# adamchang2000/DenseFusion

Measured on AMD Instinct MI355X. Metric: poses/sec (node) YCB-Video 1000 pts + 2 refine iters, higher is better.
Workload: dtype f32

## Files before the change

densefusion_amd/csrc/split_gemm.hip:

```cpp
#include "igemm.h"
#include <atomic>
#include <cstdint>
#ifdef DF_DEV
#include <map>
#include <mutex>
#include <tuple>
#endif

namespace df {
namespace {

typedef __bf16 bf16x8 __attribute__((ext_vector_type(8)));
typedef __bf16 bf16x2 __attribute__((ext_vector_type(2)));
typedef float f32x16 __attribute__((ext_vector_type(16)));
typedef float f32x2 __attribute__((ext_vector_type(2)));

constexpr int SBM = 128, SBN = 128, SBK = 32;
constexpr int PLANE_BYTES = 128 * 64;

__device__ __forceinline__ void cut3(float a0, float a1, unsigned &hi, unsigned &mid, unsigned &lo) {
  const bf16x2 h = __builtin_convertvector(f32x2{a0, a1}, bf16x2);
  hi = __builtin_bit_cast(unsigned, h);
  const float r0 = a0 - __builtin_bit_cast(float, hi << 16), r1 = a1 - __builtin_bit_cast(float, hi & 0xFFFF0000u);
  const bf16x2 m = __builtin_convertvector(f32x2{r0, r1}, bf16x2);
  mid = __builtin_bit_cast(unsigned, m);
  const float s0 = r0 - __builtin_bit_cast(float, mid << 16), s1 = r1 - __builtin_bit_cast(float, mid & 0xFFFF0000u);
  const bf16x2 l = __builtin_convertvector(f32x2{s0, s1}, bf16x2);
  lo = __builtin_bit_cast(unsigned, l);
}

__global__ void cut_planes_kernel(const float *__restrict__ w, __bf16 *__restrict__ planes, long elems, long stride) {
  const long i = (long)blockIdx.x * blockDim.x + threadIdx.x;
  if (i >= elems) return;
  unsigned h, m, l;
  cut3(w[i], 0.f, h, m, l);
  unsigned short *pl = reinterpret_cast<unsigned short *>(planes);
  pl[i] = (unsigned short)h; pl[stride + i] = (unsigned short)m; pl[2 * stride + i] = (unsigned short)l;
}

struct SplitArgs {
  const float *in; const __bf16 *wpl; const float *bias; const float *res; const float *prelu; float *out; float *colsum;
  long M, wplane;
  int N, K, in_ld, in_coff, out_ld, out_coff, res_ld, res_coff, act, rows_per_group, rows_valid, bias_group_ld;
  long z_in_coff, z_wgt, z_bias, z_out_coff;
  int tiles_m, tiles_n;
  long cs_rows;
};

__device__ __forceinline__ int piece(int row, int slot) { return row * 64 + ((slot ^ ((row >> 2) & 3)) << 4); }

__device__ __forceinline__ void split_epilogue(const SplitArgs &a, const f32x16 (&acc)[2][2], int z, long row0, int wrow, int nb, int fr, int fh, long cs_row) {
  const float slope = a.act == ACT_PRELU ? a.prelu[0] : 0.f;
  float *out = a.out + z * a.z_out_coff + a.out_coff;
  const float *bias = a.bias ? a.bias + z * a.z_bias : nullptr;
  const float *gbias = bias && a.bias_group_ld > 0 ? bias + (row0 / a.rows_per_group) * a.bias_group_ld : nullptr;
  const int grp = a.rows_per_group > 0 ? (int)(row0 / a.rows_per_group) : 0;
  const long left = a.M - row0;
  const int valid = a.rows_per_group > 0 ? a.rows_valid - (int)(row0 - (long)grp * a.rows_per_group) : (1 << 30);
  const int limit = (int)(left < valid ? left : valid);
#pragma unroll
  for (int j = 0; j < 2; ++j) {
    const int n = nb + j * 32 + fr;
    const float b1 = gbias ? gbias[n] : bias ? bias[n] : 0.f;
    float csum = 0.f;
#pragma unroll
    for (int i = 0; i < 2; ++i) {
      const int tb = wrow + i * 32 + 4 * fh;
      const long mb = row0 + tb;
      float r[16];
      if (a.res) {
#pragma unroll
        for (int e = 0; e < 16; ++e) {
          long m = mb + (e & 3) + 8 * (e >> 2);
          m = m < a.M ? m : a.M - 1;
          r[e] = a.res[m * a.res_ld + a.res_coff + n];
        }
      }
#pragma unroll
      for (int e = 0; e < 16; ++e) {
        const int tr = tb + (e & 3) + 8 * (e >> 2);
        const long m = row0 + tr;
        float v = acc[i][j][e] + b1;
        if (a.res) v += r[e];
        if (a.act == ACT_RELU) v = v > 0.f ? v : 0.f;
        else if (a.act == ACT_PRELU) v = v > 0.f ? v : v * slope;
        if (a.out && m < a.M) out[m * a.out_ld + n] = v;
        csum += tr < limit ? v : 0.f;
      }
    }
    if (a.colsum && cs_row < a.cs_rows) {
      csum += __shfl_xor(csum, 32);
      if (fh == 0) a.colsum[((size_t)z * a.cs_rows + (size_t)cs_row) * a.N + n] = csum;
    }
  }
}

__device__ __forceinline__ void split_epilogue_rows(const SplitArgs &a, const f32x16 (&acc)[2][2], int z, long row0, int wrow, int nb, int lane, long cs_row, float *blk) {
  const int fr = lane & 31, fh = lane >> 5;
  const float slope = a.act == ACT_PRELU ? a.prelu[0] : 0.f;
  const float *bias = a.bias ? a.bias + z * a.z_bias : nullptr;
  const float *gbias = bias && a.bias_group_ld > 0 ? bias + (row0 / a.rows_per_group) * a.bias_group_ld : nullptr;
  const int grp = a.rows_per_group > 0 ? (int)(row0 / a.rows_per_group) : 0;
  const long left = a.M - row0;
  const int valid = a.rows_per_group > 0 ? a.rows_valid - (int)(row0 - (long)grp * a.rows_per_group) : (1 << 30);
  const int limit = (int)(left < valid ? left : valid);
#pragma unroll
  for (int j = 0; j < 2; ++j) {
    const int n = nb + j * 32 + fr;
    const float b1 = gbias ? gbias[n] : bias ? bias[n] : 0.f;
    float csum = 0.f;
#pragma unroll
    for (int i = 0; i < 2; ++i)
#pragma unroll
      for (int e = 0; e < 16; ++e) {
        const int br = i * 32 + 4 * fh + (e & 3) + 8 * (e >> 2);
        float v = acc[i][j][e] + b1;
        if (!a.res) {
          if (a.act == ACT_RELU) v = v > 0.f ? v : 0.f;
          else if (a.act == ACT_PRELU) v = v > 0.f ? v : v * slope;
        }
        blk[br * 64 + j * 32 + fr] = v;
        csum += wrow + br < limit ? v : 0.f;
      }
    if (a.colsum && cs_row < a.cs_rows) {
      csum += __shfl_xor(csum, 32);
      if (fh == 0) a.colsum[((size_t)z * a.cs_rows + (size_t)cs_row) * a.N + n] = csum;
    }
  }
  if (!a.out) return;
  __builtin_amdgcn_fence(__ATOMIC_RELEASE, "wavefront");
  __builtin_amdgcn_wave_barrier();
  __builtin_amdgcn_fence(__ATOMIC_ACQUIRE, "wavefront");
  float *out = a.out + z * a.z_out_coff + a.out_coff;
  const int c4 = (lane & 15) * 4;
#pragma unroll 4
  for (int it = 0; it < 16; ++it) {
    const int br = it * 4 + (lane >> 4);
    const long m = row0 + wrow + br;
    float4 v = *reinterpret_cast<const float4 *>(blk + br * 64 + c4);
    if (m < a.M) {
      if (a.res) {
        const float4 r = *reinterpret_cast<const float4 *>(a.res + m * a.res_ld + a.res_coff + nb + c4);
        v.x += r.x; v.y += r.y; v.z += r.z; v.w += r.w;
        if (a.act == ACT_RELU) {
          v.x = v.x > 0.f ? v.x : 0.f; v.y = v.y > 0.f ? v.y : 0.f; v.z = v.z > 0.f ? v.z : 0.f; v.w = v.w > 0.f ? v.w : 0.f;
        } else if (a.act == ACT_PRELU) {
          v.x = v.x > 0.f ? v.x : v.x * slope; v.y = v.y > 0.f ? v.y : v.y * slope; v.z = v.z > 0.f ? v.z : v.z * slope; v.w = v.w > 0.f ? v.w : v.w * slope;
        }
      }
      *reinterpret_cast<float4 *>(out + m * a.out_ld + nb + c4) = v;
    }
  }
  __builtin_amdgcn_fence(__ATOMIC_RELEASE, "wavefront");
  __builtin_amdgcn_wave_barrier();
}

__global__ __launch_bounds__(256, 2) void gemm_split_bf16_kernel(const SplitArgs a) {
  __shared__ __attribute__((aligned(16))) unsigned char lds[6 * PLANE_BYTES];
  const int tid = threadIdx.x, lane = tid & 63, wave = tid >> 6;
  const int xcd = blockIdx.x & 7, seq = blockIdx.x >> 3;
  const int tm = (seq / a.tiles_n) * 8 + xcd, tn = seq % a.tiles_n;
  if (tm >= a.tiles_m) return;
  const int z = blockIdx.z;
  const long row0 = (long)tm * SBM;
  const int n0 = tn * SBN;
  const float *in = a.in + z * a.z_in_coff + a.in_coff;
  const __bf16 *wpl = a.wpl + z * a.z_wgt;

  const int srow0 = tid >> 2, srow1 = srow0 + 64, sslot = tid & 3;
  const int soff0 = piece(srow0, sslot), soff1 = piece(srow1, sslot);
  long r0 = row0 + srow0, r1 = row0 + srow1;
  r0 = r0 < a.M ? r0 : a.M - 1;
  r1 = r1 < a.M ? r1 : a.M - 1;
  const float *ag0 = in + r0 * a.in_ld + sslot * 8, *ag1 = in + r1 * a.in_ld + sslot * 8;
  const __bf16 *bg0 = wpl + (long)(n0 + srow0) * a.K + sslot * 8, *bg1 = wpl + (long)(n0 + srow1) * a.K + sslot * 8;
  float4 xa00, xa01, xa10, xa11, ya00, ya01, ya10, ya11;
  uint4 rb00, rb01, rb02, rb10, rb11, rb12;
#define SPLIT_FETCH_A(S, k0)                                                     \
  do {                                                                           \
    S##a00 = *reinterpret_cast<const float4 *>(ag0 + (k0));                      \
    S##a01 = *reinterpret_cast<const float4 *>(ag0 + (k0) + 4);                  \
    S##a10 = *reinterpret_cast<const float4 *>(ag1 + (k0));                      \
    S##a11 = *reinterpret_cast<const float4 *>(ag1 + (k0) + 4);                  \
  } while (0)
#define SPLIT_FETCH_B(k0)                                                        \
  do {                                                                           \
    rb00 = *reinterpret_cast<const uint4 *>(bg0 + (k0));                         \
    rb01 = *reinterpret_cast<const uint4 *>(bg0 + a.wplane + (k0));              \
    rb02 = *reinterpret_cast<const uint4 *>(bg0 + 2 * a.wplane + (k0));          \
    rb10 = *reinterpret_cast<const uint4 *>(bg1 + (k0));                         \
    rb11 = *reinterpret_cast<const uint4 *>(bg1 + a.wplane + (k0));              \
    rb12 = *reinterpret_cast<const uint4 *>(bg1 + 2 * a.wplane + (k0));          \
  } while (0)
#define SPLIT_STAGE1(x0, x1, off, b0, b1, b2)                                    \
  do {                                                                           \
    uint4 h, m, l;                                                               \
    cut3(x0.x, x0.y, h.x, m.x, l.x);                                             \
    cut3(x0.z, x0.w, h.y, m.y, l.y);                                             \
    cut3(x1.x, x1.y, h.z, m.z, l.z);                                             \
    cut3(x1.z, x1.w, h.w, m.w, l.w);                                             \
    *reinterpret_cast<uint4 *>(lds + (off)) = h;                                 \
    *reinterpret_cast<uint4 *>(lds + PLANE_BYTES + (off)) = m;                   \
    *reinterpret_cast<uint4 *>(lds + 2 * PLANE_BYTES + (off)) = l;               \
    *reinterpret_cast<uint4 *>(lds + 3 * PLANE_BYTES + (off)) = b0;              \
    *reinterpret_cast<uint4 *>(lds + 4 * PLANE_BYTES + (off)) = b1;              \
    *reinterpret_cast<uint4 *>(lds + 5 * PLANE_BYTES + (off)) = b2;              \
  } while (0)
#define SPLIT_STAGE(S)                                                           \
  do {                                                                           \
    SPLIT_STAGE1(S##a00, S##a01, soff0, rb00, rb01, rb02);                       \
    SPLIT_STAGE1(S##a10, S##a11, soff1, rb10, rb11, rb12);                       \
  } while (0)

  const int wr = wave >> 1, wc = wave & 1, fr = lane & 31, fh = lane >> 5;
  f32x16 acc[2][2];
#pragma unroll
  for (int i = 0; i < 2; ++i)
#pragma unroll
    for (int j = 0; j < 2; ++j)
#pragma unroll
      for (int e = 0; e < 16; ++e) acc[i][j][e] = 0.f;
  int offa[2][2], offb[2][2];
#pragma unroll
  for (int ks = 0; ks < 2; ++ks)
#pragma unroll
    for (int t = 0; t < 2; ++t) {
      offa[ks][t] = piece(wr * 64 + t * 32 + fr, ks * 2 + fh);
      offb[ks][t] = 3 * PLANE_BYTES + piece(wc * 64 + t * 32 + fr, ks * 2 + fh);
    }

#define SPLIT_COMPUTE()                                                                                   \
  _Pragma("unroll") for (int ks = 0; ks < 2; ++ks) {                                                      \
    bf16x8 fa[2][3], fb[2][3];                                                                            \
    _Pragma("unroll") for (int t = 0; t < 2; ++t)                                                         \
    _Pragma("unroll") for (int p = 0; p < 3; ++p) {                                                       \
      fa[t][p] = *reinterpret_cast<const bf16x8 *>(lds + p * PLANE_BYTES + offa[ks][t]);                  \
      fb[t][p] = *reinterpret_cast<const bf16x8 *>(lds + p * PLANE_BYTES + offb[ks][t]);                  \
    }                                                                                                     \
    _Pragma("unroll") for (int i = 0; i < 2; ++i)                                                         \
    _Pragma("unroll") for (int j = 0; j < 2; ++j) {                                                       \
      f32x16 c = acc[i][j];                                                        \
      c = __builtin_amdgcn_mfma_f32_32x32x16_bf16(fa[i][2], fb[j][0], c, 0, 0, 0);                        \
      c = __builtin_amdgcn_mfma_f32_32x32x16_bf16(fa[i][0], fb[j][2], c, 0, 0, 0);                        \
      c = __builtin_amdgcn_mfma_f32_32x32x16_bf16(fa[i][1], fb[j][1], c, 0, 0, 0);                        \
      c = __builtin_amdgcn_mfma_f32_32x32x16_bf16(fa[i][1], fb[j][0], c, 0, 0, 0);                        \
      c = __builtin_amdgcn_mfma_f32_32x32x16_bf16(fa[i][0], fb[j][1], c, 0, 0, 0);                        \
      c = __builtin_amdgcn_mfma_f32_32x32x16_bf16(fa[i][0], fb[j][0], c, 0, 0, 0);                        \
      acc[i][j] = c;                                                                                      \
    }                                                                                                     \
  }

  const int nk = a.K / SBK;
  SPLIT_FETCH_A(x, 0);
  SPLIT_FETCH_B(0);
  if (nk > 1) SPLIT_FETCH_A(y, SBK);
  SPLIT_STAGE(x);
  __syncthreads();
  for (int kt = 0; kt < nk; kt += 2) {
    if (kt + 1 < nk) SPLIT_FETCH_B((kt + 1) * SBK);
    if (kt + 2 < nk) SPLIT_FETCH_A(x, (kt + 2) * SBK);
    SPLIT_COMPUTE();
    if (kt + 1 >= nk) break;
    __syncthreads();
    SPLIT_STAGE(y);
    __syncthreads();
    if (kt + 2 < nk) SPLIT_FETCH_B((kt + 2) * SBK);
    if (kt + 3 < nk) SPLIT_FETCH_A(y, (kt + 3) * SBK);
    SPLIT_COMPUTE();
    if (kt + 2 >= nk) break;
    __syncthreads();
    SPLIT_STAGE(x);
    __syncthreads();
  }

  split_epilogue(a, acc, z, row0, wr * 64, n0 + wc * 64, fr, fh, (long)tm * 2 + wr);
}

constexpr int V2_APL = 256 * 64, V2_BPL = 128 * 64, V2_STAGE = 3 * V2_APL + 3 * V2_BPL;

__global__ __launch_bounds__(512, 1) void gemm_split_bf16_v2_kernel(const SplitArgs a) {
  extern __shared__ __attribute__((aligned(16))) unsigned char lds2[];
  const int tid = threadIdx.x, lane = tid & 63, wave = tid >> 6;
  const int xcd = blockIdx.x & 7, seq = blockIdx.x >> 3;
  const int tm = (seq / a.tiles_n) * 8 + xcd, tn = seq % a.tiles_n;
  if (tm >= a.tiles_m) return;
  const int z = blockIdx.z;
  const long row0 = (long)tm * 256;
  const int n0 = tn * SBN;
  const float *in = a.in + z * a.z_in_coff + a.in_coff;
  const __bf16 *wpl = a.wpl + z * a.z_wgt;

  const int srow0 = tid >> 2, srow1 = srow0 + 128, sslot = tid & 3;
  const int soff0 = piece(srow0, sslot), soff1 = piece(srow1, sslot);
  long r0 = row0 + srow0, r1 = row0 + srow1;
  r0 = r0 < a.M ? r0 : a.M - 1;
  r1 = r1 < a.M ? r1 : a.M - 1;
  const float *ag0 = in + r0 * a.in_ld + sslot * 8, *ag1 = in + r1 * a.in_ld + sslot * 8;
  const __bf16 *bg0 = wpl + (long)(n0 + srow0) * a.K + sslot * 8;
  float4 xa00, xa01, xa10, xa11, ya00, ya01, ya10, ya11;
  uint4 xb0, xb1, xb2, yb0, yb1, yb2;
#define V2_FETCH(S, k0)                                                          \
  do {                                                                           \
    S##a00 = *reinterpret_cast<const float4 *>(ag0 + (k0));                      \
    S##a01 = *reinterpret_cast<const float4 *>(ag0 + (k0) + 4);                  \
    S##a10 = *reinterpret_cast<const float4 *>(ag1 + (k0));                      \
    S##a11 = *reinterpret_cast<const float4 *>(ag1 + (k0) + 4);                  \
    S##b0 = *reinterpret_cast<const uint4 *>(bg0 + (k0));                        \
    S##b1 = *reinterpret_cast<const uint4 *>(bg0 + a.wplane + (k0));             \
    S##b2 = *reinterpret_cast<const uint4 *>(bg0 + 2 * a.wplane + (k0));         \
  } while (0)
#define V2_CUT(x0, x1, base, off)                                                \
  do {                                                                           \
    uint4 h, m, l;                                                               \
    cut3(x0.x, x0.y, h.x, m.x, l.x);                                             \
    cut3(x0.z, x0.w, h.y, m.y, l.y);                                             \
    cut3(x1.x, x1.y, h.z, m.z, l.z);                                             \
    cut3(x1.z, x1.w, h.w, m.w, l.w);                                             \
    *reinterpret_cast<uint4 *>((base) + (off)) = h;                              \
    *reinterpret_cast<uint4 *>((base) + V2_APL + (off)) = m;                     \
    *reinterpret_cast<uint4 *>((base) + 2 * V2_APL + (off)) = l;                 \
  } while (0)
#define V2_STAGE_TO(S, base)                                                     \
  do {                                                                           \
    V2_CUT(S##a00, S##a01, base, soff0);                                         \
    V2_CUT(S##a10, S##a11, base, soff1);                                         \
    *reinterpret_cast<uint4 *>((base) + 3 * V2_APL + soff0) = S##b0;             \
    *reinterpret_cast<uint4 *>((base) + 3 * V2_APL + V2_BPL + soff0) = S##b1;    \
    *reinterpret_cast<uint4 *>((base) + 3 * V2_APL + 2 * V2_BPL + soff0) = S##b2; \
  } while (0)

  const int wr = wave >> 1, wc = wave & 1, fr = lane & 31, fh = lane >> 5;
  f32x16 acc[2][2];
#pragma unroll
  for (int i = 0; i < 2; ++i)
#pragma unroll
    for (int j = 0; j < 2; ++j)
#pragma unroll
      for (int e = 0; e < 16; ++e) acc[i][j][e] = 0.f;
  int offa[2][2], offb[2][2];
#pragma unroll
  for (int ks = 0; ks < 2; ++ks)
#pragma unroll
    for (int t = 0; t < 2; ++t) {
      offa[ks][t] = piece(wr * 64 + t * 32 + fr, ks * 2 + fh);
      offb[ks][t] = 3 * V2_APL + piece(wc * 64 + t * 32 + fr, ks * 2 + fh);
    }
#define V2_COMPUTE(base)                                                                                  \
  _Pragma("unroll") for (int ks = 0; ks < 2; ++ks) {                                                      \
    bf16x8 fa[2][3], fb[2][3];                                                                            \
    _Pragma("unroll") for (int t = 0; t < 2; ++t)                                                         \
    _Pragma("unroll") for (int p = 0; p < 3; ++p) {                                                       \
      fa[t][p] = *reinterpret_cast<const bf16x8 *>((base) + p * V2_APL + offa[ks][t]);                    \
      fb[t][p] = *reinterpret_cast<const bf16x8 *>((base) + p * V2_BPL + offb[ks][t]);                    \
    }                                                                                                     \
    _Pragma("unroll") for (int q = 0; q < 6; ++q) {                                                       \
      constexpr int PA[6] = {2, 0, 1, 1, 0, 0}, PB[6] = {0, 2, 1, 0, 1, 0};                               \
      _Pragma("unroll") for (int i = 0; i < 2; ++i)                                                       \
      _Pragma("unroll") for (int j = 0; j < 2; ++j)                                                       \
        acc[i][j] = __builtin_amdgcn_mfma_f32_32x32x16_bf16(fa[i][PA[q]], fb[j][PB[q]], acc[i][j], 0, 0, 0); \
    }                                                                                                     \
  }
#define V2_BODY(FS, SS, kf, cur, nxt)                                            \
  do {                                                                           \
    V2_FETCH(FS, (kf));                                                          \
    V2_STAGE_TO(SS, nxt);                                                        \
    V2_COMPUTE(cur);                                                             \
    __builtin_amdgcn_sched_group_barrier(0x020, 7, 0);                           \
    __builtin_amdgcn_sched_group_barrier(0x100, 12, 0);                          \
    _Pragma("unroll") for (int g = 0; g < 48; ++g) {                             \
      __builtin_amdgcn_sched_group_barrier(0x008, 1, 0);                         \
      __builtin_amdgcn_sched_group_barrier(0x002, 2, 0);                         \
      if (g >= 8 && g < 32 && (g & 1) == 0) __builtin_amdgcn_sched_group_barrier(0x100, 1, 0); \
      if (g % 5 == 4) __builtin_amdgcn_sched_group_barrier(0x200, 1, 0);         \
    }                                                                            \
    __syncthreads();                                                             \
  } while (0)

  unsigned char *const st0 = lds2, *const st1 = lds2 + V2_STAGE;
  const int nk = a.K / SBK;
  const int klast = a.K - SBK;
  V2_FETCH(x, 0);
  V2_FETCH(y, SBK < klast ? SBK : klast);
  V2_STAGE_TO(x, st0);
  __syncthreads();
  int kt = 0;
  for (; kt + 1 < nk; kt += 2) {
    const int k2 = (kt + 2) * SBK, k3 = (kt + 3) * SBK;
    V2_BODY(x, y, k2 < klast ? k2 : klast, st0, st1);
    V2_BODY(y, x, k3 < klast ? k3 : klast, st1, st0);
  }
  if (nk & 1) { V2_COMPUTE(st0); }
  split_epilogue(a, acc, z, row0, wr * 64, n0 + wc * 64, fr, fh, (long)tm * 4 + wr);
}

constexpr int V3_PL = 256 * 32, V3_STAGE = 6 * V3_PL;
constexpr int V3_LDS = 8 * 64 * 64 * 4;

__device__ __forceinline__ int piece16(int row, int half) { return row * 32 + ((half ^ ((row >> 3) & 1)) << 4); }

__global__ __launch_bounds__(512, 1) void gemm_split_bf16_v3_kernel(const SplitArgs a) {
  extern __shared__ __attribute__((aligned(16))) unsigned char lds3[];
  const int tid = threadIdx.x, lane = tid & 63, wave = tid >> 6;
  const int xcd = blockIdx.x & 7, seq = blockIdx.x >> 3;
  const int tm = (seq / a.tiles_n) * 8 + xcd, tn = seq % a.tiles_n;
  if (tm >= a.tiles_m) return;
  const int z = blockIdx.z;
  const long row0 = (long)tm * 256;
  const int n0 = tn * 256;
  const float *in = a.in + z * a.z_in_coff + a.in_coff;
  const __bf16 *wpl = a.wpl + z * a.z_wgt;

  const int srow = tid >> 1, shalf = tid & 1;
  const int soff = piece16(srow, shalf);
  long r = row0 + srow;
  r = r < a.M ? r : a.M - 1;
  const float *ag = in + r * a.in_ld + shalf * 8;
  const __bf16 *bg = wpl + (long)(n0 + srow) * a.K + shalf * 8;
  float4 xa0, xa1, ya0, ya1;
  uint4 b0, b1, b2;
#define V3_FETCH_A(S, k0)                                                        \
  do {                                                                           \
    S##a0 = *reinterpret_cast<const float4 *>(ag + (k0));                        \
    S##a1 = *reinterpret_cast<const float4 *>(ag + (k0) + 4);                    \
  } while (0)
#define V3_FETCH_B(k0)                                                           \
  do {                                                                           \
    b0 = *reinterpret_cast<const uint4 *>(bg + (k0));                            \
    b1 = *reinterpret_cast<const uint4 *>(bg + a.wplane + (k0));                 \
    b2 = *reinterpret_cast<const uint4 *>(bg + 2 * a.wplane + (k0));             \
  } while (0)
#define V3_PIN(v) asm volatile("" : "+v"(v.x), "+v"(v.y), "+v"(v.z), "+v"(v.w))
#define V3_CUT0(S) do { V3_PIN(S##a0); cut3(S##a0.x, S##a0.y, ch.x, cm.x, cl.x); cut3(S##a0.z, S##a0.w, ch.y, cm.y, cl.y); } while (0)
#define V3_CUT1(S) do { V3_PIN(S##a1); cut3(S##a1.x, S##a1.y, ch.z, cm.z, cl.z); cut3(S##a1.z, S##a1.w, ch.w, cm.w, cl.w); } while (0)
#define V3_WRITE_A(base)                                                         \
  do {                                                                           \
    *reinterpret_cast<uint4 *>((base) + soff) = ch;                              \
    *reinterpret_cast<uint4 *>((base) + V3_PL + soff) = cm;                      \
    *reinterpret_cast<uint4 *>((base) + 2 * V3_PL + soff) = cl;                  \
  } while (0)
#define V3_WRITE_B(base)                                                         \
  do {                                                                           \
    *reinterpret_cast<uint4 *>((base) + 3 * V3_PL + soff) = b0;                  \
    *reinterpret_cast<uint4 *>((base) + 4 * V3_PL + soff) = b1;                  \
    *reinterpret_cast<uint4 *>((base) + 5 * V3_PL + soff) = b2;                  \
  } while (0)

  const int wr = wave >> 2, wc = wave & 3, fr = lane & 31, fh = lane >> 5;
  f32x16 acc[2][2][2];
#pragma unroll
  for (int h = 0; h < 2; ++h)
#pragma unroll
    for (int i = 0; i < 2; ++i)
#pragma unroll
      for (int j = 0; j < 2; ++j)
#pragma unroll
        for (int e = 0; e < 16; ++e) acc[h][i][j][e] = 0.f;
  const int offa = piece16(wr * 128 + fr, fh), offb = 3 * V3_PL + piece16(wc * 64 + fr, fh);
#define V3_PA(q) ((q) == 0 ? 2 : (q) == 2 || (q) == 3 ? 1 : 0)
#define V3_PB(q) ((q) == 1 ? 2 : (q) == 2 || (q) == 4 ? 1 : 0)
#define V3_READ(base, q)                                                                                  \
  do {                                                                                                    \
    _Pragma("unroll") for (int t = 0; t < 4; ++t)                                                         \
      fa[t][V3_PA(q)] = *reinterpret_cast<const bf16x8 *>((base) + V3_PA(q) * V3_PL + offa + t * 1024);   \
    _Pragma("unroll") for (int t = 0; t < 2; ++t)                                                         \
      fb[t][V3_PB(q)] = *reinterpret_cast<const bf16x8 *>((base) + V3_PB(q) * V3_PL + offb + t * 1024);   \
  } while (0)
#define V3_MFMA(q)                                                                                        \
  do {                                                                                                    \
    _Pragma("unroll") for (int i = 0; i < 4; ++i)                                                         \
    _Pragma("unroll") for (int j = 0; j < 2; ++j)                                                         \
      acc[i >> 1][i & 1][j] = __builtin_amdgcn_mfma_f32_32x32x16_bf16(fa[i][V3_PA(q)], fb[j][V3_PB(q)], acc[i >> 1][i & 1][j], 0, 0, 0); \
  } while (0)
#define V3_WEAVE(n, mask, cnt)                                                   \
  do {                                                                           \
    _Pragma("unroll") for (int g = 0; g < (n); ++g) {                            \
      __builtin_amdgcn_sched_group_barrier(0x008, 1, 0);                         \
      __builtin_amdgcn_sched_group_barrier(mask, cnt, 0);                        \
    }                                                                            \
    __builtin_amdgcn_sched_barrier(0);                                           \
  } while (0)
#define V3_BODY(FS, SS, ka, kb, cur, nxt)                                        \
  do {                                                                           \
    bf16x8 fa[4][3], fb[2][3];                                                   \
    uint4 ch, cm, cl;                                                            \
    V3_FETCH_B(kb);                                                              \
    V3_FETCH_A(FS, ka);                                                          \
    V3_READ(cur, 0);                                                             \
    __builtin_amdgcn_sched_barrier(0);                                           \
    V3_READ(cur, 1);                                                             \
    V3_MFMA(0);                                                                  \
    V3_WEAVE(6, 0x100, 1);                                                       \
    V3_READ(cur, 2);                                                             \
    V3_MFMA(1);                                                                  \
    V3_WEAVE(6, 0x100, 1);                                                       \
    V3_CUT0(SS);                                                                 \
    V3_MFMA(2);                                                                  \
    V3_WEAVE(8, 0x002, 3);                                                       \
    V3_CUT1(SS);                                                                 \
    V3_MFMA(3);                                                                  \
    V3_WEAVE(8, 0x002, 3);                                                       \
    V3_WRITE_A(nxt);                                                             \
    V3_MFMA(4);                                                                  \
    V3_WEAVE(3, 0x200, 1);                                                       \
    V3_WRITE_B(nxt);                                                             \
    V3_MFMA(5);                                                                  \
    V3_WEAVE(3, 0x200, 1);                                                       \
    __syncthreads();                                                             \
  } while (0)

  unsigned char *const st0 = lds3, *const st1 = lds3 + V3_STAGE;
  const int nk = a.K / 16;
  const int klast = a.K - 16;
  V3_FETCH_B(0);
  V3_FETCH_A(x, 0);
  V3_FETCH_A(y, 16);
  {
    uint4 ch, cm, cl;
    V3_CUT0(x);
    V3_CUT1(x);
    V3_WRITE_A(st0);
    V3_WRITE_B(st0);
  }
  __syncthreads();
  for (int s = 0; s < nk; s += 2) {
    const int k1 = (s + 1) * 16, k2 = (s + 2) * 16, k3 = (s + 3) * 16;
    V3_BODY(x, y, k2 < klast ? k2 : klast, k1, st0, st1);
    V3_BODY(y, x, k3 < klast ? k3 : klast, k2 < klast ? k2 : klast, st1, st0);
  }
  const int cs0 = tm * 4 + wr * 2;
  float *const blk = reinterpret_cast<float *>(lds3) + wave * (64 * 64);
  split_epilogue_rows(a, acc[0], z, row0, wr * 128, n0 + wc * 64, lane, (long)cs0, blk);
  split_epilogue_rows(a, acc[1], z, row0, wr * 128 + 64, n0 + wc * 64, lane, (long)cs0 + 1, blk);
}

#ifdef DF_DEV
std::mutex g_mu;
std::map<std::tuple<int, hipStream_t>, std::pair<__bf16 *, long>> g_scratch;

const __bf16 *scratch_planes(const float *w, long elems, hipStream_t st) {
  int dev = 0;
  (void)hipGetDevice(&dev);
  std::lock_guard<std::mutex> g(g_mu);
  auto &sc = g_scratch[std::make_tuple(dev, st)];
  if (sc.second < elems) {
    if (sc.first) (void)hipFree(sc.first);
    sc = {nullptr, 0};
    if (hipMalloc(reinterpret_cast<void **>(&sc.first), (size_t)elems * 3 * sizeof(__bf16)) != hipSuccess) return nullptr;
    sc.second = elems;
  }
  cut_weight_planes(w, sc.first, elems, elems, st);
  return sc.first;
}
#endif

}

int split_route(int N, int K, int epi) {
  if (N <= 0 || N % SBN != 0 || K % SBK != 0 || K < 384) return 0;
  return epi == GEMM_EPI_PLAIN || epi == GEMM_EPI_RESIDUAL || epi == GEMM_EPI_GROUPS;
}

int gemm_epi_kind(const ConvParams &p) {
  const bool groups = p.rows_per_group > 0 || p.bias_group_ld > 0 || p.colsum;
  if (p.res) return groups ? GEMM_EPI_OTHER : GEMM_EPI_RESIDUAL;
  return groups ? GEMM_EPI_GROUPS : GEMM_EPI_PLAIN;
}

void cut_weight_planes(const float *w, void *planes, long elems, long stride, hipStream_t st) {
  hipLaunchKernelGGL(cut_planes_kernel, dim3((unsigned)((elems + 255) / 256)), dim3(256), 0, st, w, reinterpret_cast<__bf16 *>(planes), elems, stride);
}

static int compute_units() {
  static std::atomic<int> cus[64];
  int dev = 0;
  (void)hipGetDevice(&dev);
  if (dev < 0 || dev >= 64) return 256;
  int n = cus[dev].load(std::memory_order_relaxed);
  if (n == 0) {
    if (hipDeviceGetAttribute(&n, hipDeviceAttributeMultiprocessorCount, dev) != hipSuccess || n <= 0) n = 256;
    cus[dev].store(n, std::memory_order_relaxed);
  }
  return n;
}

int try_split_gemm(const ConvParams &p, hipStream_t st) {
  static const bool off = dev_getenv("DF_GEMM_SPLIT_OFF") != nullptr;
  static const bool all = dev_getenv("DF_GEMM_SPLIT_BF16") != nullptr;
  static const bool verbose = dev_getenv("DF_GEMM_SPLIT_VERBOSE") != nullptr;
  if (off || p.splitk_ws || (!p.wpl && !all)) return 0;
  const long M = (long)p.B * p.OH * p.OW;
  const int K = p.Cin;
  const bool ok = p.KH == 1 && p.KW == 1 && p.stride == 1 && p.pad == 0 && p.up == 1 && p.H == p.OH && p.W == p.OW && (p.out || p.colsum) &&
                  p.Cout % SBN == 0 && K % SBK == 0 && K >= SBK && M >= 1 && gemm_epi_kind(p) != GEMM_EPI_OTHER &&
                  (p.rows_per_group == 0 ? p.bias_group_ld == 0 : p.rows_per_group % SBM == 0) && (p.z_wgt % 8) == 0;
  const bool take = ok && (all || split_route(p.Cout, K, gemm_epi_kind(p)));
  if (verbose) fprintf(stderr, "[df-split] M=%ld N=%d K=%d z%d -> %s\n", M, p.Cout, K, p.zcount, take ? "bf16 x 6" : "fp32");
  if (!take) {
    if (p.wpl && !all) return set_error(DF_ERR_ARG, "split gemm: routed launch M=%ld N=%d K=%d outside the kernels' cover", M, p.Cout, K);
    return 0;
  }
  const __bf16 *wpl = reinterpret_cast<const __bf16 *>(p.wpl);
  long wplane = p.wpl_stride;
#ifdef DF_DEV
  if (!wpl) {
    wplane = (long)(p.zcount - 1) * p.z_wgt + (long)p.Cout * K;
    wpl = scratch_planes(p.wgt, wplane, st);
    if (!wpl) return set_error(DF_ERR_LAUNCH, "split gemm: hipMalloc of the weight-plane scratch failed");
  }
#endif
  SplitArgs a{};
  a.in = p.in; a.wpl = wpl; a.bias = p.bias; a.res = p.res; a.prelu = p.prelu; a.out = p.out; a.colsum = p.colsum;
  a.M = M; a.wplane = wplane; a.N = p.Cout; a.K = K; a.in_ld = p.in_ld; a.in_coff = p.in_coff; a.out_ld = p.out_ld; a.out_coff = p.out_coff;
  a.res_ld = p.res_ld; a.res_coff = p.res_coff; a.act = p.act; a.rows_per_group = p.rows_per_group; a.rows_valid = p.rows_valid; a.bias_group_ld = p.bias_group_ld;
  a.z_in_coff = p.z_in_coff; a.z_wgt = p.z_wgt; a.z_bias = p.z_bias; a.z_out_coff = p.z_out_coff;
  a.cs_rows = ((M + 127) / 128) * 2;
  a.tiles_n = p.Cout / SBN;
  static const int variant = dev_getenv("DF_GEMM_SPLIT_V") ? atoi(dev_getenv("DF_GEMM_SPLIT_V")) : 3;
  const bool v2 = variant >= 2 && K >= 384 && (p.rows_per_group == 0 || p.rows_per_group % 256 == 0);
  const long tiles3 = ((M + 255) / 256) * (p.Cout / 256) * p.zcount;
  const bool rows16 = (!p.out || (reinterpret_cast<uintptr_t>(p.out) % 16 == 0 && p.out_ld % 4 == 0 && p.out_coff % 4 == 0 && p.z_out_coff % 4 == 0)) &&
                      (!p.res || (reinterpret_cast<uintptr_t>(p.res) % 16 == 0 && p.res_ld % 4 == 0 && p.res_coff % 4 == 0));
  const bool v3 = v2 && variant >= 3 && p.Cout % 256 == 0 && rows16 && tiles3 >= compute_units();
  if (verbose) fprintf(stderr, "[df-split]   form %s\n", v3 ? "256x256" : v2 ? "256x128" : "128x128");
  if (v3) {
    const int rc = raise_lds_limit(reinterpret_cast<const void *>(&gemm_split_bf16_v3_kernel), V3_LDS);
    if (rc != DF_OK) return rc;
    a.tiles_m = (int)((M + 255) / 256);
    a.tiles_n = p.Cout / 256;
    const unsigned grid = (unsigned)(((a.tiles_m + 7) / 8) * 8 * a.tiles_n);
    hipLaunchKernelGGL(gemm_split_bf16_v3_kernel, dim3(grid, 1, p.zcount), dim3(512), V3_LDS, st, a);
  } else if (v2) {
    const int rc = raise_lds_limit(reinterpret_cast<const void *>(&gemm_split_bf16_v2_kernel), 2 * V2_STAGE);
    if (rc != DF_OK) return rc;
    a.tiles_m = (int)((M + 255) / 256);
    const unsigned grid = (unsigned)(((a.tiles_m + 7) / 8) * 8 * a.tiles_n);
    hipLaunchKernelGGL(gemm_split_bf16_v2_kernel, dim3(grid, 1, p.zcount), dim3(512), 2 * V2_STAGE, st, a);
  } else {
    a.tiles_m = (int)((M + SBM - 1) / SBM);
    const unsigned grid = (unsigned)(((a.tiles_m + 7) / 8) * 8 * a.tiles_n);
    hipLaunchKernelGGL(gemm_split_bf16_kernel, dim3(grid, 1, p.zcount), dim3(256), 0, st, a);
  }
  return 1;
}

}
```

Baseline: 10290.

## Make 256x256 split-bf16 GEMM persistent with cross-tile prefetch and branchless epilogue

Turns the v3 split-bf16 GEMM into a persistent kernel. The grid is sized to the compute-unit count and each workgroup loops over tiles across z. The first A/B fetch of the next tile is issued during the last k-step of the current one, so its load latency overlaps the tail and epilogue, and per-tile launch and ramp-up cost is meant to shrink. The epilogue becomes branchless for activations and gets a separate no-residual store loop, with bias hoisted. It also adds an optional start-skew sleep and a dev-only timeline probe, at the cost of more code complexity and possible load imbalance from static tile striding.

```diff
diff --git a/densefusion_amd/csrc/split_gemm.hip b/densefusion_amd/csrc/split_gemm.hip
--- a/densefusion_amd/csrc/split_gemm.hip
+++ b/densefusion_amd/csrc/split_gemm.hip
@@ -2,6 +2,7 @@
 #include <atomic>
 #include <cstdint>
 #ifdef DF_DEV
+#include <vector>
 #include <map>
 #include <mutex>
 #include <tuple>
@@ -45,6 +46,9 @@
   long z_in_coff, z_wgt, z_bias, z_out_coff;
   int tiles_m, tiles_n;
   long cs_rows;
+  int zcount;
+  int skew_p, skew_naps, pgrid;
+  unsigned long long *tl;
 };
 
 __device__ __forceinline__ int piece(int row, int slot) { return row * 64 + ((slot ^ ((row >> 2) & 3)) << 4); }
@@ -95,11 +99,17 @@
   }
 }
 
-__device__ __forceinline__ void split_epilogue_rows(const SplitArgs &a, const f32x16 (&acc)[2][2], int z, long row0, int wrow, int nb, int lane, long cs_row, float *blk) {
+__device__ __forceinline__ float split_bias(const SplitArgs &a, int z, long row0, int n) {
+  const float *bias = a.bias ? a.bias + z * a.z_bias : nullptr;
+  const float *gbias = bias && a.bias_group_ld > 0 ? bias + (row0 / a.rows_per_group) * a.bias_group_ld : nullptr;
+  return gbias ? gbias[n] : bias ? bias[n] : 0.f;
+}
+
+__device__ __forceinline__ void split_epilogue_rows(const SplitArgs &a, const f32x16 (&acc)[2][2], int z, long row0, int wrow, int nb, int lane, long cs_row, float *blk, const float (&bj)[2]) {
   const int fr = lane & 31, fh = lane >> 5;
   const float slope = a.act == ACT_PRELU ? a.prelu[0] : 0.f;
-  const float *bias = a.bias ? a.bias + z * a.z_bias : nullptr;
-  const float *gbias = bias && a.bias_group_ld > 0 ? bias + (row0 / a.rows_per_group) * a.bias_group_ld : nullptr;
+  const bool relu = a.act == ACT_RELU, prelu = a.act == ACT_PRELU;
+  const bool relu0 = relu && !a.res, prelu0 = prelu && !a.res;
   const int grp = a.rows_per_group > 0 ? (int)(row0 / a.rows_per_group) : 0;
   const long left = a.M - row0;
   const int valid = a.rows_per_group > 0 ? a.rows_valid - (int)(row0 - (long)grp * a.rows_per_group) : (1 << 30);
@@ -107,7 +117,7 @@
 #pragma unroll
   for (int j = 0; j < 2; ++j) {
     const int n = nb + j * 32 + fr;
-    const float b1 = gbias ? gbias[n] : bias ? bias[n] : 0.f;
+    const float b1 = bj[j];
     float csum = 0.f;
 #pragma unroll
     for (int i = 0; i < 2; ++i)
@@ -115,10 +125,9 @@
       for (int e = 0; e < 16; ++e) {
         const int br = i * 32 + 4 * fh + (e & 3) + 8 * (e >> 2);
         float v = acc[i][j][e] + b1;
-        if (!a.res) {
-          if (a.act == ACT_RELU) v = v > 0.f ? v : 0.f;
-          else if (a.act == ACT_PRELU) v = v > 0.f ? v : v * slope;
-        }
+        float neg = prelu0 ? v * slope : v;
+        neg = relu0 ? 0.f : neg;
+        v = v > 0.f ? v : neg;
         blk[br * 64 + j * 32 + fr] = v;
         csum += wrow + br < limit ? v : 0.f;
       }
@@ -133,22 +142,29 @@
   __builtin_amdgcn_fence(__ATOMIC_ACQUIRE, "wavefront");
   float *out = a.out + z * a.z_out_coff + a.out_coff;
   const int c4 = (lane & 15) * 4;
+  if (!a.res) {
 #pragma unroll 4
-  for (int it = 0; it < 16; ++it) {
-    const int br = it * 4 + (lane >> 4);
-    const long m = row0 + wrow + br;
-    float4 v = *reinterpret_cast<const float4 *>(blk + br * 64 + c4);
-    if (m < a.M) {
-      if (a.res) {
+    for (int it = 0; it < 16; ++it) {
+      const int br = it * 4 + (lane >> 4);
+      const long m = row0 + wrow + br;
+      const float4 v = *reinterpret_cast<const float4 *>(blk + br * 64 + c4);
+      if (m < a.M) *reinterpret_cast<float4 *>(out + m * a.out_ld + nb + c4) = v;
+    }
+  } else {
+#pragma unroll 4
+    for (int it = 0; it < 16; ++it) {
+      const int br = it * 4 + (lane >> 4);
+      const long m = row0 + wrow + br;
+      float4 v = *reinterpret_cast<const float4 *>(blk + br * 64 + c4);
+      if (m < a.M) {
         const float4 r = *reinterpret_cast<const float4 *>(a.res + m * a.res_ld + a.res_coff + nb + c4);
         v.x += r.x; v.y += r.y; v.z += r.z; v.w += r.w;
-        if (a.act == ACT_RELU) {
-          v.x = v.x > 0.f ? v.x : 0.f; v.y = v.y > 0.f ? v.y : 0.f; v.z = v.z > 0.f ? v.z : 0.f; v.w = v.w > 0.f ? v.w : 0.f;
-        } else if (a.act == ACT_PRELU) {
-          v.x = v.x > 0.f ? v.x : v.x * slope; v.y = v.y > 0.f ? v.y : v.y * slope; v.z = v.z > 0.f ? v.z : v.z * slope; v.w = v.w > 0.f ? v.w : v.w * slope;
-        }
+        float4 neg = v;
+        if (prelu) { neg.x = v.x * slope; neg.y = v.y * slope; neg.z = v.z * slope; neg.w = v.w * slope; }
+        if (relu) neg = float4{0.f, 0.f, 0.f, 0.f};
+        v.x = v.x > 0.f ? v.x : neg.x; v.y = v.y > 0.f ? v.y : neg.y; v.z = v.z > 0.f ? v.z : neg.z; v.w = v.w > 0.f ? v.w : neg.w;
+        *reinterpret_cast<float4 *>(out + m * a.out_ld + nb + c4) = v;
       }
-      *reinterpret_cast<float4 *>(out + m * a.out_ld + nb + c4) = v;
     }
   }
   __builtin_amdgcn_fence(__ATOMIC_RELEASE, "wavefront");
@@ -394,40 +410,51 @@
 }
 
 constexpr int V3_PL = 256 * 32, V3_STAGE = 6 * V3_PL;
+constexpr int V3_SKEW = 0;
 constexpr int V3_LDS = 8 * 64 * 64 * 4;
 
 __device__ __forceinline__ int piece16(int row, int half) { return row * 32 + ((half ^ ((row >> 3) & 1)) << 4); }
 
+template <bool PERSIST, bool TL>
 __global__ __launch_bounds__(512, 1) void gemm_split_bf16_v3_kernel(const SplitArgs a) {
   extern __shared__ __attribute__((aligned(16))) unsigned char lds3[];
   const int tid = threadIdx.x, lane = tid & 63, wave = tid >> 6;
-  const int xcd = blockIdx.x & 7, seq = blockIdx.x >> 3;
-  const int tm = (seq / a.tiles_n) * 8 + xcd, tn = seq % a.tiles_n;
-  if (tm >= a.tiles_m) return;
-  const int z = blockIdx.z;
-  const long row0 = (long)tm * 256;
-  const int n0 = tn * 256;
-  const float *in = a.in + z * a.z_in_coff + a.in_coff;
-  const __bf16 *wpl = a.wpl + z * a.z_wgt;
+  const int xcd = blockIdx.x & 7;
+  const int rx = (a.tiles_m - xcd + 7) >> 3;
+  const int per_z = rx * a.tiles_n;
+  const int vstep = gridDim.x >> 3, vend = PERSIST ? per_z * a.zcount : 0;
+  int v = blockIdx.x >> 3;
+  if (PERSIST ? v >= vend : v >= per_z) return;
+  if (!PERSIST) v += blockIdx.z * per_z;
+  int z = v / per_z, tm = ((v - z * per_z) / a.tiles_n) * 8 + xcd, tn = (v - z * per_z) % a.tiles_n;
+  long row0 = (long)tm * 256;
+  int n0 = tn * 256;
 
   const int srow = tid >> 1, shalf = tid & 1;
   const int soff = piece16(srow, shalf);
-  long r = row0 + srow;
-  r = r < a.M ? r : a.M - 1;
-  const float *ag = in + r * a.in_ld + shalf * 8;
-  const __bf16 *bg = wpl + (long)(n0 + srow) * a.K + shalf * 8;
+  const float *ag;
+  const __bf16 *bg;
+#define V3_POINT_A(srow_, shalf_)                                                     \
+  do {                                                                           \
+    long r = row0 + (srow_);                                                     \
+    r = r < a.M ? r : a.M - 1;  \
+    ag = a.in + z * a.z_in_coff + a.in_coff + r * a.in_ld + (shalf_) * 8;        \
+  } while (0)
+#define V3_POINT_B(srow_, shalf_) bg = a.wpl + z * a.z_wgt + (long)(n0 + (srow_)) * a.K + (shalf_) * 8
+  V3_POINT_A(srow, shalf);
+  V3_POINT_B(srow, shalf);
   float4 xa0, xa1, ya0, ya1;
   uint4 b0, b1, b2;
-#define V3_FETCH_A(S, k0)                                                        \
-  do {                                                                           \
-    S##a0 = *reinterpret_cast<const float4 *>(ag + (k0));                        \
-    S##a1 = *reinterpret_cast<const float4 *>(ag + (k0) + 4);                    \
-  } while (0)
-#define V3_FETCH_B(k0)                                                           \
-  do {                                                                           \
-    b0 = *reinterpret_cast<const uint4 *>(bg + (k0));                            \
-    b1 = *reinterpret_cast<const uint4 *>(bg + a.wplane + (k0));                 \
-    b2 = *reinterpret_cast<const uint4 *>(bg + 2 * a.wplane + (k0));             \
+#define V3_FETCH_A(S, pa)                                                        \
+  do {                                                                           \
+    S##a0 = *reinterpret_cast<const float4 *>(pa);                               \
+    S##a1 = *reinterpret_cast<const float4 *>((pa) + 4);                         \
+  } while (0)
+#define V3_FETCH_B(pb)                                                           \
+  do {                                                                           \
+    b0 = *reinterpret_cast<const uint4 *>(pb);                                   \
+    b1 = *reinterpret_cast<const uint4 *>((pb) + a.wplane);                      \
+    b2 = *reinterpret_cast<const uint4 *>((pb) + 2 * a.wplane);                  \
   } while (0)
 #define V3_PIN(v) asm volatile("" : "+v"(v.x), "+v"(v.y), "+v"(v.z), "+v"(v.w))
 #define V3_CUT0(S) do { V3_PIN(S##a0); cut3(S##a0.x, S##a0.y, ch.x, cm.x, cl.x); cut3(S##a0.z, S##a0.w, ch.y, cm.y, cl.y); } while (0)
@@ -447,14 +474,6 @@
 
   const int wr = wave >> 2, wc = wave & 3, fr = lane & 31, fh = lane >> 5;
   f32x16 acc[2][2][2];
-#pragma unroll
-  for (int h = 0; h < 2; ++h)
-#pragma unroll
-    for (int i = 0; i < 2; ++i)
-#pragma unroll
-      for (int j = 0; j < 2; ++j)
-#pragma unroll
-        for (int e = 0; e < 16; ++e) acc[h][i][j][e] = 0.f;
   const int offa = piece16(wr * 128 + fr, fh), offb = 3 * V3_PL + piece16(wc * 64 + fr, fh);
 #define V3_PA(q) ((q) == 0 ? 2 : (q) == 2 || (q) == 3 ? 1 : 0)
 #define V3_PB(q) ((q) == 1 ? 2 : (q) == 2 || (q) == 4 ? 1 : 0)
@@ -479,12 +498,13 @@
     }                                                                            \
     __builtin_amdgcn_sched_barrier(0);                                           \
   } while (0)
-#define V3_BODY(FS, SS, ka, kb, cur, nxt)                                        \
+#define V3_BODY(FS, SS, pa, pb, cur, nxt)                                        \
   do {                                                                           \
     bf16x8 fa[4][3], fb[2][3];                                                   \
     uint4 ch, cm, cl;                                                            \
-    V3_FETCH_B(kb);                                                              \
-    V3_FETCH_A(FS, ka);                                                          \
+    V3_FETCH_B(pb);                                                              \
+    __builtin_amdgcn_sched_barrier(0);  \
+    V3_FETCH_A(FS, pa);                                                          \
     V3_READ(cur, 0);                                                             \
     __builtin_amdgcn_sched_barrier(0);                                           \
     V3_READ(cur, 1);                                                             \
@@ -507,30 +527,98 @@
     V3_WEAVE(3, 0x200, 1);                                                       \
     __syncthreads();                                                             \
   } while (0)
+#define V3_LAST(FS, pa, pb, cur)                                                 \
+  do {                                                                           \
+    bf16x8 fa[4][3], fb[2][3];                                                   \
+    V3_FETCH_B(pb);                                                              \
+    __builtin_amdgcn_sched_barrier(0);                                           \
+    V3_FETCH_A(FS, pa);                                                          \
+    V3_READ(cur, 0);                                                             \
+    __builtin_amdgcn_sched_barrier(0);                                           \
+    V3_READ(cur, 1);                                                             \
+    V3_MFMA(0);                                                                  \
+    V3_WEAVE(6, 0x100, 1);                                                       \
+    V3_READ(cur, 2);                                                             \
+    V3_MFMA(1);                                                                  \
+    V3_WEAVE(6, 0x100, 1);                                                       \
+    V3_MFMA(2);                                                                  \
+    V3_MFMA(3);                                                                  \
+    V3_MFMA(4);                                                                  \
+    V3_MFMA(5);                                                                  \
+    __builtin_amdgcn_sched_barrier(0);                                           \
+    __syncthreads();                                                             \
+  } while (0)
 
   unsigned char *const st0 = lds3, *const st1 = lds3 + V3_STAGE;
   const int nk = a.K / 16;
-  const int klast = a.K - 16;
-  V3_FETCH_B(0);
-  V3_FETCH_A(x, 0);
-  V3_FETCH_A(y, 16);
-  {
-    uint4 ch, cm, cl;
-    V3_CUT0(x);
-    V3_CUT1(x);
-    V3_WRITE_A(st0);
-    V3_WRITE_B(st0);
-  }
-  __syncthreads();
-  for (int s = 0; s < nk; s += 2) {
-    const int k1 = (s + 1) * 16, k2 = (s + 2) * 16, k3 = (s + 3) * 16;
-    V3_BODY(x, y, k2 < klast ? k2 : klast, k1, st0, st1);
-    V3_BODY(y, x, k3 < klast ? k3 : klast, k2 < klast ? k2 : klast, st1, st0);
-  }
-  const int cs0 = tm * 4 + wr * 2;
   float *const blk = reinterpret_cast<float *>(lds3) + wave * (64 * 64);
-  split_epilogue_rows(a, acc[0], z, row0, wr * 128, n0 + wc * 64, lane, (long)cs0, blk);
-  split_epilogue_rows(a, acc[1], z, row0, wr * 128 + 64, n0 + wc * 64, lane, (long)cs0 + 1, blk);
+  if (a.skew_p > 1 && blockIdx.z == 0 && blockIdx.x < a.pgrid) {
+    const int naps = ((blockIdx.x >> 3) % a.skew_p) * a.skew_naps;
+    for (int i = 0; i < naps; ++i) __builtin_amdgcn_s_sleep(16);
+  }
+  V3_FETCH_B(bg);
+  V3_FETCH_A(x, ag);
+  V3_FETCH_A(y, ag + 16);
+  for (;;) {
+#pragma unroll
+    for (int h = 0; h < 2; ++h)
+#pragma unroll
+      for (int i = 0; i < 2; ++i)
+#pragma unroll
+        for (int j = 0; j < 2; ++j)
+#pragma unroll
+          for (int e = 0; e < 16; ++e) acc[h][i][j][e] = 0.f;
+    {
+      uint4 ch, cm, cl;
+      V3_CUT0(x);
+      V3_CUT1(x);
+      V3_WRITE_A(st0);
+      V3_WRITE_B(st0);
+    }
+    __syncthreads();
+    unsigned long long t0 = 0, t1 = 0;
+    if (TL) t0 = __builtin_amdgcn_s_memrealtime();
+    const int zc = z, tmc = tm;
+    const long row0c = row0;
+    const int n0c = n0, vc = v;
+    v += vstep;
+    const bool more = PERSIST && v < vend;
+    int s = 0;
+    for (; s + 2 < nk; s += 2) {
+      const int k1 = (s + 1) * 16, k2 = (s + 2) * 16, k3 = (s + 3) * 16;
+      V3_BODY(x, y, ag + k2, bg + k1, st0, st1);
+      V3_BODY(y, x, ag + k3, bg + k2, st1, st0);
+    }
+    if (more) {
+      z = v / per_z;
+      tm = ((v - z * per_z) / a.tiles_n) * 8 + xcd;
+      tn = (v - z * per_z) % a.tiles_n;
+      row0 = (long)tm * 256;
+      n0 = tn * 256;
+    }
+    int nsrow = srow;
+    asm volatile("" : "+v"(nsrow));
+    bg += (s + 1) * 16;
+    V3_POINT_A(nsrow, shalf);
+    V3_BODY(x, y, ag, bg, st0, st1);
+    V3_POINT_B(nsrow, shalf);
+    V3_LAST(y, ag + 16, bg, st1);
+    if (TL) t1 = __builtin_amdgcn_s_memrealtime();
+    float bj[2];
+#pragma unroll
+    for (int j = 0; j < 2; ++j) bj[j] = split_bias(a, zc, row0c, n0c + wc * 64 + j * 32 + fr);
+    const int cs0 = tmc * 4 + wr * 2;
+    int elane = lane, ewrow = wr * 128;
+    asm volatile("" : "+v"(elane), "+v"(ewrow));
+    split_epilogue_rows(a, acc[0], zc, row0c, ewrow, n0c + wc * 64, elane, (long)cs0, blk, bj);
+    split_epilogue_rows(a, acc[1], zc, row0c, ewrow + 64, n0c + wc * 64, elane, (long)cs0 + 1, blk, bj);
+    if (TL && tid == 0) {
+      unsigned long long *t = a.tl + ((size_t)vc * 8 + xcd) * 4;
+      t[0] = t0; t[1] = t1; t[2] = __builtin_amdgcn_s_memrealtime(); t[3] = blockIdx.x;
+    }
+    if (!more) break;
+    __syncthreads();
+  }
 }
 
 #ifdef DF_DEV
@@ -581,6 +669,38 @@
     cus[dev].store(n, std::memory_order_relaxed);
   }
   return n;
+}
+
+static int launch_v3(SplitArgs &a, bool persist, unsigned pgrid, unsigned grid, hipStream_t st) {
+  auto go = [&](auto kernel, dim3 g) {
+    const int rc = raise_lds_limit(reinterpret_cast<const void *>(kernel), V3_LDS);
+    if (rc != DF_OK) return rc;
+    hipLaunchKernelGGL(kernel, g, dim3(512), V3_LDS, st, a);
+    return 1;
+  };
+#ifdef DF_DEV
+  static const char *const tl_path = dev_getenv("DF_GEMM_SPLIT_TIMELINE");
+  if (tl_path) {
+    const size_t words = (size_t)grid * a.zcount * 4;
+    if (hipMalloc(reinterpret_cast<void **>(&a.tl), words * 8) != hipSuccess) return set_error(DF_ERR_LAUNCH, "split gemm: hipMalloc of the timeline failed");
+    (void)hipMemsetAsync(a.tl, 0, words * 8, st);
+    const int rc = persist ? go(&gemm_split_bf16_v3_kernel<true, true>, dim3(pgrid)) : go(&gemm_split_bf16_v3_kernel<false, true>, dim3(grid, 1, a.zcount));
+    std::vector<unsigned long long> host(words);
+    (void)hipStreamSynchronize(st);
+    (void)hipMemcpy(host.data(), a.tl, words * 8, hipMemcpyDeviceToHost);
+    (void)hipFree(a.tl);
+    if (FILE *f = fopen(tl_path, "a")) {
+      fprintf(f, "launch M=%ld N=%d K=%d z=%d persist=%d skew=%d\n", a.M, a.N, a.K, a.zcount, (int)persist, a.skew_p);
+      for (size_t i = 0; i < words; i += 4)
+        if (host[i]) fprintf(f, "%llu %llu %llu %llu\n", host[i + 3], host[i], host[i + 1], host[i + 2]);
+      fclose(f);
+    }
+    return rc;
+  }
+  if (!persist) return go(&gemm_split_bf16_v3_kernel<false, false>, dim3(grid, 1, a.zcount));
+#endif
+  (void)persist; (void)grid;
+  return go(&gemm_split_bf16_v3_kernel<true, false>, dim3(pgrid));
 }
 
 int try_split_gemm(const ConvParams &p, hipStream_t st) {
@@ -616,6 +736,10 @@
   a.cs_rows = ((M + 127) / 128) * 2;
   a.tiles_n = p.Cout / SBN;
   static const int variant = dev_getenv("DF_GEMM_SPLIT_V") ? atoi(dev_getenv("DF_GEMM_SPLIT_V")) : 3;
+  static const bool persist = !dev_getenv("DF_GEMM_SPLIT_PERSIST") || atoi(dev_getenv("DF_GEMM_SPLIT_PERSIST")) != 0;
+  static const int skew = dev_getenv("DF_GEMM_SPLIT_SKEW") ? atoi(dev_getenv("DF_GEMM_SPLIT_SKEW")) : V3_SKEW;
+  a.skew_p = skew;
+  a.skew_naps = skew > 1 ? (int)(K * 0.14 / 0.43 / skew) : 0;
   const bool v2 = variant >= 2 && K >= 384 && (p.rows_per_group == 0 || p.rows_per_group % 256 == 0);
   const long tiles3 = ((M + 255) / 256) * (p.Cout / 256) * p.zcount;
   const bool rows16 = (!p.out || (reinterpret_cast<uintptr_t>(p.out) % 16 == 0 && p.out_ld % 4 == 0 && p.out_coff % 4 == 0 && p.z_out_coff % 4 == 0)) &&
@@ -623,12 +747,13 @@
   const bool v3 = v2 && variant >= 3 && p.Cout % 256 == 0 && rows16 && tiles3 >= compute_units();
   if (verbose) fprintf(stderr, "[df-split]   form %s\n", v3 ? "256x256" : v2 ? "256x128" : "128x128");
   if (v3) {
-    const int rc = raise_lds_limit(reinterpret_cast<const void *>(&gemm_split_bf16_v3_kernel), V3_LDS);
-    if (rc != DF_OK) return rc;
     a.tiles_m = (int)((M + 255) / 256);
     a.tiles_n = p.Cout / 256;
+    a.zcount = p.zcount;
+    const unsigned pgrid = (unsigned)((compute_units() + 7) / 8 * 8);
     const unsigned grid = (unsigned)(((a.tiles_m + 7) / 8) * 8 * a.tiles_n);
-    hipLaunchKernelGGL(gemm_split_bf16_v3_kernel, dim3(grid, 1, p.zcount), dim3(512), V3_LDS, st, a);
+    a.pgrid = (int)pgrid;
+    return launch_v3(a, persist, pgrid, grid, st);
   } else if (v2) {
     const int rc = raise_lds_limit(reinterpret_cast<const void *>(&gemm_split_bf16_v2_kernel), 2 * V2_STAGE);
     if (rc != DF_OK) return rc;
```

Result: faster. 10390 (median of 6 runs) (+1.0%).
